# ShangHua-Gao/SOD100K

Hardware: NVIDIA H100
Metric: images/sec CSNet fwd 224x224 (higher is better)
Workload: dtype fp16

## Files before the change

### sod100k_b200/csrc/il_stream.cuh

```cuda
#pragma once
#include <cuda.h>

#include "il_block.cuh"

namespace csnet {

constexpr int kIlsMaxThreads = 384;
constexpr int kIlsMaxC = 64;
constexpr int kIlsHiStages = 2, kIlsLoStages = 3;

struct IlsArgs {
  void* yh;
  void* yl;
  const uint32_t* wh;
  const uint32_t* wl;
  DwParams dw1h, dw1l, dw2h, dw2l;
  float bias_h[kIlsMaxC], sm1_h[kIlsMaxC], bias_l[kIlsMaxC], sm1_l[kIlsMaxC];
  int32_t N, H, W;
  int32_t Chi, Cli, Cho, Clo;
  int32_t K8, K16, NH, NL;
  int32_t SH, SL, ST;
  int32_t GH, GL;
  int32_t ns, gsn, hl;
  int32_t GR, GLR;
  int32_t Ci, BW;
  int32_t off_xlo;
  int32_t cpi, total_chunks;
  int32_t dw_warps;
  int32_t hi_stage_bytes, lo_stage_bytes;
  int32_t off_xl, off_xh, off_t1l, off_wbh, off_wbl, off_bar, off_zero, off_epi, off_dwp, smem_bytes;
};

__device__ __forceinline__ void tma_load_5d(uint32_t dst, const CUtensorMap* tm, uint32_t bar, int c0, int c1, int c2, int c3, int c4) {
  asm volatile("cp.async.bulk.tensor.5d.shared::cluster.global.mbarrier::complete_tx::bytes [%0], [%1, {%3, %4, %5, %6, %7}], [%2];\n"
               ::"r"(dst), "l"(tm), "r"(bar), "r"(c0), "r"(c1), "r"(c2), "r"(c3), "r"(c4) : "memory");
}
__device__ __forceinline__ void tma_load_4d_a(uint32_t dst, const CUtensorMap* tm, uint32_t bar, int c0, int c1, int c2, int c3) {
  asm volatile("cp.async.bulk.tensor.4d.shared::cluster.global.mbarrier::complete_tx::bytes [%0], [%1, {%3, %4, %5, %6}], [%2];\n"
               ::"r"(dst), "l"(tm), "r"(bar), "r"(c0), "r"(c1), "r"(c2), "r"(c3) : "memory");
}
__device__ __forceinline__ void mbar_expect_tx_a(uint32_t bar, uint32_t bytes) {
  asm volatile("mbarrier.arrive.expect_tx.shared::cta.b64 _, [%0], %1;\n" ::"r"(bar), "r"(bytes) : "memory");
}
__device__ __forceinline__ void mbar_wait_a(uint32_t bar, uint32_t parity) {
  uint32_t ok = 0;
  const long long t0 = clock64();
  while (true) {
    asm volatile("{\n.reg .pred p;\nmbarrier.try_wait.parity.shared::cta.b64 p, [%1], %2;\nselp.u32 %0, 1, 0, p;\n}\n"
                 : "=r"(ok) : "r"(bar), "r"(parity) : "memory");
    if (ok) break;
    if (clock64() - t0 > 4000000000LL) __trap();
  }
}
__device__ __forceinline__ uint64_t gmma_desc(uint32_t saddr, uint32_t lbo_bytes, uint32_t sbo_bytes) {
// ... 51 lines not shown
                 : "l"(da), "l"(db), "r"(acc));
  }
  static __device__ __forceinline__ void mma0(float (&d)[32], uint64_t da, uint64_t db) {
    asm volatile("{\n.reg .pred p;\nsetp.ne.b32 p, %34, 0;\n"
                 "wgmma.mma_async.sync.aligned.m64n64k16.f32.f16.f16 {%0, %1, %2, %3, %4, %5, %6, %7, %8, %9, %10, %11, %12, %13, %14, %15, %16, %17, %18, %19, %20, %21, %22, %23, %24, %25, %26, %27, %28, %29, %30, %31}, %32, %33, p, 1, 1, 1, 0;\n}\n"
                 : "=f"(d[0]), "=f"(d[1]), "=f"(d[2]), "=f"(d[3]), "=f"(d[4]), "=f"(d[5]), "=f"(d[6]), "=f"(d[7]), "=f"(d[8]), "=f"(d[9]), "=f"(d[10]), "=f"(d[11]), "=f"(d[12]), "=f"(d[13]), "=f"(d[14]), "=f"(d[15]), "=f"(d[16]), "=f"(d[17]), "=f"(d[18]), "=f"(d[19]), "=f"(d[20]), "=f"(d[21]), "=f"(d[22]), "=f"(d[23]), "=f"(d[24]), "=f"(d[25]), "=f"(d[26]), "=f"(d[27]), "=f"(d[28]), "=f"(d[29]), "=f"(d[30]), "=f"(d[31])
                 : "l"(da), "l"(db), "r"(0u));
  }
};
template <> struct Wgmma<80> {
  static __device__ __forceinline__ void mma(float (&d)[40], uint64_t da, uint64_t db, uint32_t acc) {
    asm volatile("{\n.reg .pred p;\nsetp.ne.b32 p, %42, 0;\n"
                 "wgmma.mma_async.sync.aligned.m64n80k16.f32.f16.f16 {%0, %1, %2, %3, %4, %5, %6, %7, %8, %9, %10, %11, %12, %13, %14, %15, %16, %17, %18, %19, %20, %21, %22, %23, %24, %25, %26, %27, %28, %29, %30, %31, %32, %33, %34, %35, %36, %37, %38, %39}, %40, %41, p, 1, 1, 1, 0;\n}\n"
                 : "+f"(d[0]), "+f"(d[1]), "+f"(d[2]), "+f"(d[3]), "+f"(d[4]), "+f"(d[5]), "+f"(d[6]), "+f"(d[7]), "+f"(d[8]), "+f"(d[9]), "+f"(d[10]), "+f"(d[11]), "+f"(d[12]), "+f"(d[13]), "+f"(d[14]), "+f"(d[15]), "+f"(d[16]), "+f"(d[17]), "+f"(d[18]), "+f"(d[19]), "+f"(d[20]), "+f"(d[21]), "+f"(d[22]), "+f"(d[23]), "+f"(d[24]), "+f"(d[25]), "+f"(d[26]), "+f"(d[27]), "+f"(d[28]), "+f"(d[29]), "+f"(d[30]), "+f"(d[31]), "+f"(d[32]), "+f"(d[33]), "+f"(d[34]), "+f"(d[35]), "+f"(d[36]), "+f"(d[37]), "+f"(d[38]), "+f"(d[39])
                 : "l"(da), "l"(db), "r"(acc));
  }
  static __device__ __forceinline__ void mma0(float (&d)[40], uint64_t da, uint64_t db) {
    asm volatile("{\n.reg .pred p;\nsetp.ne.b32 p, %42, 0;\n"
                 "wgmma.mma_async.sync.aligned.m64n80k16.f32.f16.f16 {%0, %1, %2, %3, %4, %5, %6, %7, %8, %9, %10, %11, %12, %13, %14, %15, %16, %17, %18, %19, %20, %21, %22, %23, %24, %25, %26, %27, %28, %29, %30, %31, %32, %33, %34, %35, %36, %37, %38, %39}, %40, %41, p, 1, 1, 1, 0;\n}\n"
                 : "=f"(d[0]), "=f"(d[1]), "=f"(d[2]), "=f"(d[3]), "=f"(d[4]), "=f"(d[5]), "=f"(d[6]), "=f"(d[7]), "=f"(d[8]), "=f"(d[9]), "=f"(d[10]), "=f"(d[11]), "=f"(d[12]), "=f"(d[13]), "=f"(d[14]), "=f"(d[15]), "=f"(d[16]), "=f"(d[17]), "=f"(d[18]), "=f"(d[19]), "=f"(d[20]), "=f"(d[21]), "=f"(d[22]), "=f"(d[23]), "=f"(d[24]), "=f"(d[25]), "=f"(d[26]), "=f"(d[27]), "=f"(d[28]), "=f"(d[29]), "=f"(d[30]), "=f"(d[31]), "=f"(d[32]), "=f"(d[33]), "=f"(d[34]), "=f"(d[35]), "=f"(d[36]), "=f"(d[37]), "=f"(d[38]), "=f"(d[39])
                 : "l"(da), "l"(db), "r"(0u));
  }
};
__device__ __forceinline__ void wgmma_fence() { asm volatile("wgmma.fence.sync.aligned;\n" ::: "memory"); }
__device__ __forceinline__ void wgmma_commit_wait() {
  asm volatile("wgmma.commit_group.sync.aligned;\n" ::: "memory");
  asm volatile("wgmma.wait_group.sync.aligned 0;\n" ::: "memory");
}
__device__ __forceinline__ void warpgroup_bar(int wg) { asm volatile("bar.sync %0, 128;\n" ::"r"(1 + wg) : "memory"); }
template <int N>
__device__ __forceinline__ void wgmma_block(float (&d)[N / 2], uint64_t da, uint64_t db, int K16) {
  wgmma_fence();
  Wgmma<N>::mma0(d, da, db);
  for (int ks = 1; ks < (K16 >> 4); ++ks) Wgmma<N>::mma(d, da + (uint64_t)(16 * ks), db + (uint64_t)(16 * ks), 1u);
  wgmma_commit_wait();
}
__device__ __forceinline__ uint32_t lds32(uint32_t a) { uint32_t v; asm volatile("ld.shared.b32 %0, [%1];\n" : "=r"(v) : "r"(a)); return v; }
__device__ __forceinline__ uint2 lds64(uint32_t a) { uint2 v; asm volatile("ld.shared.v2.b32 {%0, %1}, [%2];\n" : "=r"(v.x), "=r"(v.y) : "r"(a)); return v; }
__device__ __forceinline__ uint4 lds128(uint32_t a) {
  uint4 v;
  asm volatile("ld.shared.v4.b32 {%0, %1, %2, %3}, [%4];\n" : "=r"(v.x), "=r"(v.y), "=r"(v.z), "=r"(v.w) : "r"(a));
  return v;
}
__device__ __forceinline__ uint16_t lds16(uint32_t a) { uint16_t v; asm volatile("ld.shared.u16 %0, [%1];\n" : "=h"(v) : "r"(a)); return v; }
__device__ __forceinline__ void sts128(uint32_t a, uint4 v) {
  asm volatile("st.shared.v4.b32 [%0], {%1, %2, %3, %4};\n" ::"r"(a), "r"(v.x), "r"(v.y), "r"(v.z), "r"(v.w) : "memory");
}
__device__ __forceinline__ void sts16(uint32_t a, uint16_t v) { asm volatile("st.shared.u16 [%0], %1;\n" ::"r"(a), "h"(v) : "memory"); }

__device__ __forceinline__ uint16_t h16(const uint32_t* row, int j) { return (j & 1) ? (uint16_t)(row[j >> 1] >> 16) : (uint16_t)row[j >> 1]; }

constexpr int kIlsDwpBytes = 96;
constexpr int kIlsTX = 20, kIlsT2 = 18, kIlsTO = 16;

template <int NO, bool kStart = false>
__device__ __forceinline__ void ils_dw_taps(float (&acc)[NO], const float* row, float4 w) {
#pragma unroll
  for (int i = 0; i < NO; ++i) {
    acc[i] = fmaf(row[i], w.x, kStart ? w.w : acc[i]);
// ... 46 lines not shown
  const float4 v1 = ils_dw_param(prm + 64u);
  ils_dw_taps<kIlsTO>(sob, q, v1);
  if (make_out) {
    uint32_t o[8];
#pragma unroll
    for (int k = 0; k < kIlsTO; k += 2) o[k >> 1] = Pack<T>::from_f2(prelu_m1(soa[k], v1.w), prelu_m1(soa[k + 1], v1.w));
    *reinterpret_cast<uint4*>(out) = make_uint4(o[0], o[1], o[2], o[3]);
    if (e.outB) *reinterpret_cast<uint4*>(out + 8) = make_uint4(o[4], o[5], o[6], o[7]);
  }
  ils_dw_taps<kIlsTO, true>(soa, q, ils_dw_param(prm + 48u));
  ils_dw_taps<kIlsT2, true>(s2a, x, ils_dw_param(prm));
}
template <typename T>
__device__ __forceinline__ void ils_dw_load(float (&x)[kIlsTX], uint32_t pA, uint32_t pB, uint32_t pL, uint32_t pR) {
  const uint4 a = lds128(pA), b = lds128(pB);
  const uint32_t u[10] = {lds32(pL), a.x, a.y, a.z, a.w, b.x, b.y, b.z, b.w, lds32(pR)};
#pragma unroll
  for (int i = 0; i < 10; ++i) {
    const float2 f = Pack<T>::to_f2(u[i]);
    x[2 * i] = f.x; x[2 * i + 1] = f.y;
  }
}

__device__ __forceinline__ void stsm_x4_trans(uint32_t addr, uint32_t a, uint32_t b, uint32_t c, uint32_t d) {
  asm volatile("stmatrix.sync.aligned.m8n8.x4.trans.shared.b16 [%0], {%1, %2, %3, %4};\n" ::"r"(addr), "r"(a), "r"(b), "r"(c), "r"(d) : "memory");
}

template <typename T, int N>
__device__ __forceinline__ void ils_block(uint64_t da, uint64_t db, int K16, int wg, uint32_t tile, uint32_t gstride, int g0, int ngroups,
                                          uint32_t eb, uint32_t es, uint32_t dummy, int lane) {
  float d[N / 2];
  wgmma_block<N>(d, da, db, K16);
  warpgroup_bar(wg);
  const int q = lane & 3, mrow = lane & 7, mat = lane >> 3;
#pragma unroll
  for (int cc = 0; cc < N / 16; ++cc) {
    const uint32_t co = (uint32_t)(cc * 16 + 2 * q) * 4u;
    const uint2 bA = lds64(eb + co), bB = lds64(eb + co + 32u), sA = lds64(es + co), sB = lds64(es + co + 32u);
    const float b0 = __uint_as_float(bA.x), b1 = __uint_as_float(bA.y), b2 = __uint_as_float(bB.x), b3 = __uint_as_float(bB.y);
    const float s0 = __uint_as_float(sA.x), s1 = __uint_as_float(sA.y), s2 = __uint_as_float(sB.x), s3 = __uint_as_float(sB.y);
    const float* r = d + 8 * cc;
    const uint32_t m0 = Pack<T>::from_f2(prelu_m1(r[0] + b0, s0), prelu_m1(r[1] + b1, s1));
    const uint32_t m1 = Pack<T>::from_f2(prelu_m1(r[2] + b0, s0), prelu_m1(r[3] + b1, s1));
    const uint32_t m2 = Pack<T>::from_f2(prelu_m1(r[4] + b2, s2), prelu_m1(r[5] + b3, s3));
    const uint32_t m3 = Pack<T>::from_f2(prelu_m1(r[6] + b2, s2), prelu_m1(r[7] + b3, s3));
    const int pg = g0 + (mat & 1);
    const uint32_t addr = pg < ngroups ? tile + (uint32_t)pg * gstride + (uint32_t)(cc * 16 + 8 * (mat >> 1) + mrow) * 16u
                                       : dummy + (uint32_t)(mat * 8 + mrow) * 16u;
    stsm_x4_trans(addr, m0, m1, m2, m3);
  }
}
template <typename T>
__device__ __forceinline__ void ils_block_n(int N, uint64_t da, uint64_t db, int K16, int wg, uint32_t tile, uint32_t gstride, int g0,
                                            int ngroups, uint32_t eb, uint32_t es, uint32_t dummy, int lane) {
  switch (N) {
    case 16: ils_block<T, 16>(da, db, K16, wg, tile, gstride, g0, ngroups, eb, es, dummy, lane); break;
    case 32: ils_block<T, 32>(da, db, K16, wg, tile, gstride, g0, ngroups, eb, es, dummy, lane); break;
    case 48: ils_block<T, 48>(da, db, K16, wg, tile, gstride, g0, ngroups, eb, es, dummy, lane); break;
    default: ils_block<T, 64>(da, db, K16, wg, tile, gstride, g0, ngroups, eb, es, dummy, lane); break;
  }
}

template <typename T, bool kStem = false>
__global__ void __launch_bounds__(kIlsMaxThreads, 1)
il_stream_kernel(const __grid_constant__ IlsArgs A, const __grid_constant__ CUtensorMap tmH, const __grid_constant__ CUtensorMap tmL) {
  extern __shared__ uint8_t smem_raw[];
  const int tid = threadIdx.x, lane = tid & 31, warp = tid >> 5, nthreads = blockDim.x, nwarps = nthreads >> 5;
  const uint32_t sbase = (smem_u32(smem_raw) + 127u) & ~127u;
  const uint32_t XL = sbase + A.off_xl, XH = sbase + A.off_xh, T1L = sbase + A.off_t1l, WBH = sbase + A.off_wbh,
                 WBL = sbase + A.off_wbl, BAR = sbase + A.off_bar, ZERO = sbase + A.off_zero;
  uint8_t* gbase = smem_raw + (sbase - smem_u32(smem_raw));
  const uint32_t bar_h = BAR, bar_l = BAR + 16;
  const uint32_t EPI = sbase + A.off_epi, DUMMY = EPI + 1024;

  const int H = A.H, W = A.W, Hl = H >> 1, Wl = W >> 1;
  const int Chi = A.Chi, Cli = A.Cli, Cho = A.Cho, Clo = A.Clo;
  const int GH = A.GH, GL = A.GL, SH = A.SH, SL = A.SL, ST = A.ST, NH = A.NH, NL = A.NL, K16 = A.K16;
  const int GR = A.GR, GLR = A.GLR, hl = A.hl, gsn = A.gsn;
  const int cpi = A.cpi;

  if (tid == 0) {
    for (int i = 0; i < 6; ++i) asm volatile("mbarrier.init.shared::cta.b64 [%0], 1;\n" ::"r"(BAR + 8 * i) : "memory");
// ... 45 lines not shown
  __syncthreads();

  const int n_hi_tasks = Cho * (gsn >> 1);
  const bool dw_hi = tid < n_hi_tasks;
  const int dwt = dw_hi ? tid : tid - n_hi_tasks;
  const int Gs = dw_hi ? gsn : gsn >> 1;
  const int Gd = (Gs + 1) >> 1, Cd = dw_hi ? Cho : Clo, Sd = dw_hi ? SH : ST;
  const bool dw_live = dwt < Cd * Gd;
  const int dc = dw_live ? dwt / Gd : 0, dg = dw_live ? 2 * (dwt - dc * Gd) : 0;
  const uint32_t prm = sbase + A.off_dwp + (uint32_t)((dw_hi ? dc : Cho + dc) * kIlsDwpBytes);
  const int dw_rows = dw_hi ? 4 : 2;
  const int dHd = dw_hi ? H : Hl, dWd = dw_hi ? W : Wl;
  const uint32_t dw_off = (uint32_t)((dg + hl) * Sd + dc) * 16u, dw_rowstep = (uint32_t)((dw_hi ? GR : GLR) * Sd) * 16u;
  const int Gimg = dw_hi ? GH : GL;

  const int nbh = (4 * GR + 7) >> 3, nbl = NL > 0 ? (2 * GLR + 7) >> 3 : 0;
  const uint64_t db_h = gmma_desc(WBH, 128u, (uint32_t)(K16 >> 3) * 128u), db_l = gmma_desc(WBL, 128u, (uint32_t)(K16 >> 3) * 128u);
  const uint32_t hi_tx = (uint32_t)(64 * SH * GR), lo_tx = kStem ? (uint32_t)(A.BW * 4 * A.Ci * 4) : (uint32_t)(32 * SL * GLR);
  const uint32_t XLO = sbase + A.off_xlo;

  int ra = (int)((long long)blockIdx.x * A.total_chunks / gridDim.x);
  const int rb = (int)((long long)(blockIdx.x + 1) * A.total_chunks / gridDim.x);
  uint32_t hq = 0, lq = 0;

  while (ra < rb) {
    const int item = ra / cpi, ca = ra - item * cpi;
    const int n = item / A.ns, gs0 = (item - n * A.ns) * gsn;
    const int cb = (ca + (rb - ra)) < cpi ? (ca + (rb - ra)) : cpi;
    ra += cb - ca;
    const int c0 = ca > 0 ? ca - 1 : 0, c1 = cb < cpi ? cb : cpi - 1;
    const int cl0 = c0 > 0 ? c0 - 1 : 0, cl1 = c1 + 1 < cpi ? c1 + 1 : cpi - 1;
    const int out_lo = dw_hi ? 4 * ca : 2 * ca, out_hi = dw_hi ? 4 * cb : 2 * cb;
    const uint32_t hq0 = hq, lq0 = lq;
    hq += (uint32_t)(c1 - c0 + 1);
    lq += (uint32_t)(cl1 - cl0 + 1);
    auto hi_stage = [&](int c) { return XH + ((hq0 + (uint32_t)(c - c0)) & 1u) * (uint32_t)A.hi_stage_bytes; };
    auto lo_stage = [&](int cl) { return XL + ((lq0 + (uint32_t)(cl - cl0)) % 3u) * (uint32_t)A.lo_stage_bytes; };
    auto issue_hi = [&](int c) {
      const uint32_t q = hq0 + (uint32_t)(c - c0), bar = bar_h + 8 * (q & 1u);
      mbar_expect_tx_a(bar, hi_tx);
      tma_load_5d(hi_stage(c), &tmH, bar, 0, 0, gs0 - hl, 4 * c, n);
    };
    auto issue_lo = [&](int cl) {
      const uint32_t q = lq0 + (uint32_t)(cl - cl0), bar = bar_l + 8 * (q % 3u);
      mbar_expect_tx_a(bar, lo_tx);
      if (kStem) tma_load_4d_a(lo_stage(cl), &tmL, bar, 8 * (gs0 - hl) - 4, 4 * cl, 0, n);
      else tma_load_5d(lo_stage(cl), &tmL, bar, 0, 0, (gs0 >> 1) - hl, 2 * cl, n);
    };
    if (tid == 0) {
      asm volatile("fence.proxy.async.shared::cta;\n" ::: "memory");
      if (!kStem) {
        issue_hi(c0);
        if (c0 + 1 <= c1) issue_hi(c0 + 1);
      }
      for (int cl = cl0; cl <= cl1 && cl <= c0 + 1; ++cl) issue_lo(cl);
    }
    int lo_waited = 0;
    IlsTail tl;
    if (dw_live) ils_dw_start(tl, prm);
    const int gimg = (dw_hi ? gs0 : gs0 >> 1) + dg;
    const bool hasB = gimg + 1 < Gimg, zeroL = gimg == 0, zeroR = gimg + 2 >= Gimg || dg + 2 >= Gs + hl;
    IlsTaskEdges edg;
    edg.m0 = zeroL ? 0.f : 1.f;
    edg.m9 = hasB ? 1.f : 0.f;
    edg.m17 = gimg + 2 >= Gimg ? 0.f : 1.f;
    edg.outB = dg + 1 < Gs;
    const uint32_t sd = (uint32_t)Sd * 16u;
    uint16_t* ybase = reinterpret_cast<uint16_t*>(dw_hi ? A.yh : A.yl) + ((size_t)n * Cd + dc) * dHd * dWd + 8 * gimg;

    for (int c = c0; c <= c1; ++c) {
      {
        const uint32_t q = hq0 + (uint32_t)(c - c0);
        if (!kStem) mbar_wait_a(bar_h + 8 * (q & 1u), (q >> 1) & 1u);
        const int need = (c + 1 < cpi ? c + 1 : cpi - 1) - cl0 + 1;
        while (lo_waited < need) {
          const uint32_t ql = lq0 + (uint32_t)lo_waited;
          mbar_wait_a(bar_l + 8 * (ql % 3u), (ql / 3u) & 1u);
          ++lo_waited;
        }
      }
      const uint32_t xh = hi_stage(c), xl = kStem ? XLO : lo_stage(c);
      if (kStem) {
        const int Ci = A.Ci, BW = A.BW;
        const int n_hi = 4 * GR * Ci * 3, n_lo = Clo > 0 ? 2 * GLR * Ci * 3 : 0;
        for (int task = tid; task < n_hi + n_lo; task += nthreads) {
          const bool hb = task < n_hi;
          const int t = hb ? task : task - n_hi, Gt = hb ? GR : GLR;
          const int ck = t % (Ci * 3), rg = t / (Ci * 3);
          const int ci = ck / 3, ky = ck - ci * 3, r = rg / Gt, g = rg - r * Gt;
          float f[10];
          if (hb) {
            const int yy = 4 * c + r + ky - 1;
            if (yy >= 0 && yy < H) {
              const uint32_t a = lo_stage(yy >> 2) + (uint32_t)(((ci * 4 + (yy & 3)) * BW + 8 * g + 3) * 4);
              const uint4 m0 = lds128(a + 4u), m1 = lds128(a + 20u);
              f[0] = __uint_as_float(lds32(a)); f[9] = __uint_as_float(lds32(a + 36u));
              f[1] = __uint_as_float(m0.x); f[2] = __uint_as_float(m0.y); f[3] = __uint_as_float(m0.z); f[4] = __uint_as_float(m0.w);
              f[5] = __uint_as_float(m1.x); f[6] = __uint_as_float(m1.y); f[7] = __uint_as_float(m1.z); f[8] = __uint_as_float(m1.w);
            } else {
#pragma unroll
              for (int j = 0; j < 10; ++j) f[j] = 0.f;
            }
          } else {
// ... 71 lines not shown
            const int ga = 2 * glr - hl;
            const bool okA = ga >= 0, okB = ga + 1 < GR;
            const uint32_t src = xh + (uint32_t)(ga * SH + ch) * 16u;
            const uint32_t dst = xl + (uint32_t)(glr * SL + Cli + ch) * 16u;
#pragma unroll
            for (int lr = 0; lr < 2; ++lr) {
              const uint32_t r0 = src + (uint32_t)(2 * lr * GR * SH) * 16u, r1 = r0 + (uint32_t)(GR * SH) * 16u;
              const uint4 a0 = lds128(okA ? r0 : ZERO), a1 = lds128(okB ? r0 + (uint32_t)SH * 16u : ZERO), c0_ = lds128(okA ? r1 : ZERO),
                          c1_ = lds128(okB ? r1 + (uint32_t)SH * 16u : ZERO);
              auto hmax = [](uint32_t u, uint32_t v) {
                return __byte_perm(Pack<T>::max2(u, __byte_perm(u, 0u, 0x1032)), Pack<T>::max2(v, __byte_perm(v, 0u, 0x1032)), 0x5410);
              };
              uint4 o;
              o.x = hmax(Pack<T>::max2(a0.x, c0_.x), Pack<T>::max2(a0.y, c0_.y));
              o.y = hmax(Pack<T>::max2(a0.z, c0_.z), Pack<T>::max2(a0.w, c0_.w));
              o.z = hmax(Pack<T>::max2(a1.x, c1_.x), Pack<T>::max2(a1.y, c1_.y));
              o.w = hmax(Pack<T>::max2(a1.z, c1_.z), Pack<T>::max2(a1.w, c1_.w));
              sts128(dst + (uint32_t)(lr * GLR * SL) * 16u, o);
            }
          }
        }
      }
      asm volatile("fence.proxy.async.shared::cta;\n" ::: "memory");
      __syncthreads();
      if (warp == nwarps - 1 && lane == 0) {
        asm volatile("fence.proxy.async.shared::cta;\n" ::: "memory");
        if (!kStem && c >= c0 + 1 && c + 1 <= c1) issue_hi(c + 1);
        if (c + 2 <= cl1) issue_lo(c + 2);
      }
      if (warp < (nwarps & ~3)) {
        const int wg = warp >> 2, qd = warp & 3, wgs = nwarps >> 2;
        for (int b = wg; b < nbh + nbl; b += wgs) {
          if (b < nbh)
            ils_block_n<T>(NH, gmma_desc(xh + (uint32_t)(b * 8 * SH) * 16u, 128u, (uint32_t)SH * 16u), db_h, K16, wg, xh, (uint32_t)SH * 16u,
                           b * 8 + qd * 2, 4 * GR, EPI, EPI + 256u, DUMMY, lane);
          else
            ils_block_n<T>(NL, gmma_desc(xl + (uint32_t)((b - nbh) * 8 * SL) * 16u, 128u, (uint32_t)SL * 16u), db_l, K16, wg, T1L,
                           (uint32_t)ST * 16u, (b - nbh) * 8 + qd * 2, 2 * GLR, EPI + 512u, EPI + 768u, DUMMY, lane);
        }
      }
      __syncthreads();
      if (dw_live) {
        const uint32_t t1b = (dw_hi ? xh : T1L) + dw_off;
        auto row = [&](float (&a2)[kIlsT2], float (&b2)[kIlsT2], float (&ao)[kIlsTO], float (&bo)[kIlsTO], int rr) {
          const int r = dw_rows * c + rr, tr = r - 1, orow = r - 2;
          const bool make_t2 = tr >= 0 && tr >= out_lo - 1 && tr <= out_hi;
          const bool make_out = orow >= out_lo && orow < out_hi;
          const uint32_t p = t1b + (uint32_t)rr * dw_rowstep;
          float x[kIlsTX];
          ils_dw_load<T>(x, p, hasB ? p + sd : ZERO, zeroL ? ZERO : p - sd + 12u, zeroR ? ZERO : p + 2u * sd);
          ils_dw_push<T>(a2, b2, ao, bo, x, prm, make_t2, edg, make_out, ybase + (size_t)orow * dWd);
        };
        for (int rr = 0; rr < dw_rows; rr += 2) {
          row(tl.s2a, tl.s2b, tl.soa, tl.sob, rr);
          row(tl.s2b, tl.s2a, tl.sob, tl.soa, rr + 1);
        }
      }
    }
    if (cb == cpi && dw_live) {
      float z[kIlsTX];
#pragma unroll
      for (int i = 0; i < kIlsTX; ++i) z[i] = 0.f;
      ils_dw_push<T>(tl.s2a, tl.s2b, tl.soa, tl.sob, z, prm, true, edg, dHd - 2 >= out_lo, ybase + (size_t)(dHd - 2) * dWd);
      ils_dw_push<T>(tl.s2b, tl.s2a, tl.sob, tl.soa, z, prm, false, edg, dHd - 1 >= out_lo, ybase + (size_t)(dHd - 1) * dWd);
    }
    __syncthreads();
  }
}

}
```

### sod100k_b200/csrc/plan.cu

```cuda
#include <cuda.h>
#include <cuda_runtime.h>

#include <cstdio>
#include <cstdlib>
#include <cstring>
#include <cstdint>
#include <new>
#include <string>
#include <vector>

#include "../../include/csnet_b200.h"
#include "generic_ops.cuh"
#include "il_block.cuh"
#include "il_stream.cuh"
#include "mix_stream.cuh"
#include "ms_direct.cuh"
#include "mix_tc.cuh"
#include "dw_fast.cuh"
#include "image_io.cuh"
#include "resize.cuh"
#include "resize_adj.cuh"

namespace {

// ... 465 lines not shown
  A.H = Yh.H; A.W = Yh.W;
  A.Chi = stem ? Xh.C * 9 : Xh.C; A.Cli = stem ? 0 : Xl.C; A.Cho = Yh.C; A.Clo = op.dst2 >= 0 ? P.tensors[op.dst2].C : 0;
  A.Ci = stem ? Xh.C : 0;
  if (stem && (Xh.dtype != CSNET_F32 || A.Chi > 32 || A.W % 4)) return false;
  if (A.W % 16 || A.H % 4 || A.Cho > csnet::kIlsMaxC || A.Clo > csnet::kIlsMaxC || A.Chi + A.Cli > 64) return false;
  A.K8 = stem ? 32 : round_up(A.Chi + A.Cli, 8);
  A.K16 = round_up(A.Chi + A.Cli, 16);
  A.NH = round_up(A.Cho, 16);
  A.NL = A.Clo > 0 ? round_up(A.Clo, 16) : 0;
  A.GH = A.W / 8; A.GL = A.W / 16;
  A.SH = (A.K16 > A.NH ? A.K16 : A.NH) + 1;
  A.SL = A.Clo > 0 ? A.K16 + 1 : (A.Cli | 1);
  A.ST = A.NL + 1;
  A.cpi = A.H / 4;
  auto r128 = [](int v) { return (v + 127) / 128 * 128; };
  bool found = false;
  csnet::IlsArgs best{};
  for (int ns = 1; ns <= 16; ++ns) {
    if (P.ils_force_ns > 0 && ns != P.ils_force_ns) continue;
    if (A.GH % ns || (A.GH / ns) % 2) continue;
    csnet::IlsArgs T = A;
    T.ns = ns; T.gsn = A.GH / ns; T.hl = ns > 1 ? 1 : 0;
    T.GR = T.gsn + 2 * T.hl; T.GLR = T.gsn / 2 + 2 * T.hl;
    T.dw_warps = (T.Cho * (T.gsn / 2) + T.Clo * ((T.gsn / 2 + 1) / 2) + 31) / 32;
    if (T.dw_warps < 4) T.dw_warps = 4;
    const int warps = T.dw_warps;
    if (warps * 32 > csnet::kIlsMaxThreads || T.SH > 256 || T.SL > 256 || T.GR > 256) continue;
    const int nbh = (4 * T.GR + 7) / 8, nbl = T.Clo > 0 ? (2 * T.GLR + 7) / 8 : 0;
    T.BW = 8 * T.GR + 8;
    if (stem && T.BW > 256) continue;
    T.lo_stage_bytes = stem ? r128(T.BW * 4 * T.Ci * 4) : r128(2 * T.GLR * T.SL * 16);
    T.hi_stage_bytes = r128(4 * T.GR * T.SH * 16);
    T.off_xl = 0;
    T.off_xh = csnet::kIlsLoStages * T.lo_stage_bytes;
    T.off_t1l = T.off_xh + csnet::kIlsHiStages * T.hi_stage_bytes;
    T.off_wbh = T.off_t1l + r128(2 * T.GLR * T.ST * 16);
    T.off_wbl = T.off_wbh + r128(T.NH * T.K16 * 2);
    T.off_bar = T.off_wbl + r128(T.NL * T.K16 * 2);
    T.off_zero = T.off_bar + 256;
    T.off_epi = T.off_zero + 128;
    T.off_dwp = T.off_epi + 1536;
    T.off_xlo = T.off_dwp + r128((T.Cho + T.Clo) * csnet::kIlsDwpBytes);
    int end = T.off_xlo + (stem ? r128(2 * T.GLR * T.SL * 16) : 0);
    const int over_h = T.off_xh + T.hi_stage_bytes + nbh * 8 * T.SH * 16,
              over_l = (stem ? T.off_xlo : T.off_xl + 2 * T.lo_stage_bytes) + nbl * 8 * T.SL * 16;
    end = over_h > end ? over_h : end;
    end = over_l > end ? over_l : end;
    T.smem_bytes = end + 128;
// ... 484 lines not shown
      break;
    }
    case Kern::Gn: {
      const csnet_tensor_desc& S = P->tensors[op.paths[0].src];
      csnet::GnArgs A{};
      A.src = P->tensor_ptr(op.paths[0].src, N, ext_ptrs);
      A.dst = P->tensor_ptr(op.dst, N, ext_ptrs);
      A.gamma = P->blob + op.ext_off[0];
      A.beta = P->blob + op.ext_off[1];
      A.slope = op.slope_off >= 0 ? P->blob + op.slope_off : nullptr;
      A.stats = P->gn_stats;
      A.src_dtype = S.dtype; A.dst_dtype = D.dtype; A.C = D.C; A.HW = D.H * D.W; A.groups = op.paths[0].up;
      gn_stats_kernel<<<dim3(A.groups, N), kThreads, 0, stream>>>(A);
      const int bx = (A.HW + kThreads * 4 - 1) / (kThreads * 4);
      gn_apply_kernel<<<dim3(bx < 1 ? 1 : bx, D.C, N), kThreads, 0, stream>>>(A);
      break;
    }
    case Kern::IlStream: {
      csnet::IlsArgs A = R.ils;
      A.yh = P->tensor_ptr(op.dst, N, ext_ptrs);
      A.yl = op.dst2 >= 0 ? P->tensor_ptr(op.dst2, N, ext_ptrs) : nullptr;
      A.N = N;
      A.total_chunks = N * A.ns * A.cpi;
      CUtensorMap tmH, tmL;
      const bool stem = A.Ci > 0;
      if (stem) {
        if (!encode_image_map(&tmL, P->tensor_ptr(op.paths[0].src, N, ext_ptrs), N, A.Ci, A.H, A.W, A.BW, 4, A.Ci))
          return fail(CSNET_E_CUDA, "cuTensorMapEncodeTiled failed (streaming ILBlock, image)");
        tmH = tmL;
      } else if (!encode_group_map(&tmH, P->tensor_ptr(op.paths[0].src, N, ext_ptrs), N, A.Chi, A.H, A.W, A.SH, A.GR, 4) ||
                 !encode_group_map(&tmL, P->tensor_ptr(op.paths[1].src, N, ext_ptrs), N, A.Cli, A.H / 2, A.W / 2, A.SL, A.GLR, 2))
        return fail(CSNET_E_CUDA, "cuTensorMapEncodeTiled failed (streaming ILBlock)");
      int grid = A.total_chunks / 4;
      grid = grid < 1 ? 1 : (grid > P->num_sms ? P->num_sms : grid);
      if (stem) csnet::il_stream_kernel<__half, true><<<grid, A.dw_warps * 32, A.smem_bytes, stream>>>(A, tmH, tmL);
      else csnet::il_stream_kernel<__half, false><<<grid, A.dw_warps * 32, A.smem_bytes, stream>>>(A, tmH, tmL);
      break;
    }
    case Kern::IlBlock: {
      csnet::IlArgs A = R.il;
      A.xh = P->tensor_ptr(op.paths[0].src, N, ext_ptrs);
      if (!A.first) A.xl = P->tensor_ptr(op.paths[1].src, N, ext_ptrs);
      A.yh = P->tensor_ptr(op.dst, N, ext_ptrs);
      if (op.dst2 >= 0) A.yl = P->tensor_ptr(op.dst2, N, ext_ptrs);
      const int tiles_y = (A.H + A.TH - 1) / A.TH;
      dim3 grid(A.tiles_x * tiles_y, 1, N);
// ... 126 lines not shown
}

void* csnet_plan_tensor_ptr(csnet_plan* P, int32_t tensor, int32_t N) {
  if (!P || tensor < 0 || tensor >= (int)P->tensors.size() || N <= 0 || N > P->max_batch) return nullptr;
  if (P->tensors[tensor].external >= 0) return nullptr;
  return P->tensor_ptr(tensor, N, nullptr);
}

int csnet_plan_read_tensor(csnet_plan* P, int32_t tensor, int32_t N, void* dst, void* stream) {
  void* src = csnet_plan_tensor_ptr(P, tensor, N);
  if (!src || !dst) return fail(CSNET_E_INVALID, "csnet_plan_read_tensor: bad tensor / batch / destination");
  const csnet_tensor_desc& d = P->tensors[tensor];
  DeviceGuard guard_(P->device);
  CU_CHECK(cudaMemcpyAsync(dst, src, (size_t)N * d.C * d.H * d.W * dtype_size(d.dtype), cudaMemcpyDeviceToDevice,
                           (cudaStream_t)stream));
  return CSNET_OK;
}

const char* csnet_plan_op_kernel(const csnet_plan* P, int32_t i) {
  if (!P || i < 0 || i >= (int32_t)P->ops.size()) return "";
  return kKernNames[(int)P->launch[i].kern];
}

int32_t csnet_plan_launches(const csnet_plan* P) {
  if (!P) return 0;
  int32_t n = 0;
  for (size_t i = 0; i < P->ops.size(); ++i)
    n += P->launch[i].kern == Kern::Gn ? 2 : (P->launch[i].kern == Kern::Msd ? P->ops[i].n_paths : 1);
  return n;
}

int64_t csnet_plan_arena_bytes(const csnet_plan* P) { return P ? P->arena_per_image * (int64_t)P->max_batch : 0; }

void csnet_plan_destroy(csnet_plan* P) {
  if (!P) return;
  drop_graphs(P);
  if (P->cap_stream) cudaStreamDestroy(P->cap_stream);
  DeviceGuard guard_(P->device);
  if (P->blob) cudaFree(P->blob);
  if (P->arena) cudaFree(P->arena);
  if (P->gn_stats) cudaFree(P->gn_stats);
  for (const OpLaunch& R : P->launch)
    for (uint16_t* q : R.w16)
      if (q) cudaFree(q);
  for (int b = 0; b < 2; ++b) {
    if (P->h_in[b]) cudaFree(P->h_in[b]);
// ... 326 lines not shown
```

Before: 18440.

## Switch streaming ILBlock GEMM to register-A wgmma via transposed ldmatrix

Replaces the shared-memory-descriptor wgmma for the A operand with register-sourced wgmma, loading A fragments per k-step with ldmatrix.trans. The block loop is split into separate hi and lo passes with their own warpgroup strides, and dw_warps is rounded up to a multiple of four so every warp joins a warpgroup. Compile-time-gated phase timing instrumentation is also added. Each k-step now does commit/wait serially, which may cost tensor-core overlap in exchange for avoiding the smem A layout constraint.

```diff
diff --git a/sod100k_b200/csrc/il_stream.cuh b/sod100k_b200/csrc/il_stream.cuh
--- a/sod100k_b200/csrc/il_stream.cuh
+++ b/sod100k_b200/csrc/il_stream.cuh
@@ -29,7 +29,24 @@
   int32_t dw_warps;
   int32_t hi_stage_bytes, lo_stage_bytes;
   int32_t off_xl, off_xh, off_t1l, off_wbh, off_wbl, off_bar, off_zero, off_epi, off_dwp, smem_bytes;
-};
+#ifdef CSNET_ILS_PHASES
+  int32_t phase_slot;
+#endif
+};
+
+#ifdef CSNET_ILS_PHASES
+enum IlsPhase { kPhWait, kPhResample, kPhBarA, kPhGemm, kPhBarB, kPhTail, kPhPiece, kIlsPhases };
+constexpr int kIlsPhaseSlots = 128;
+__device__ unsigned long long g_ils_phase[kIlsPhaseSlots][2][kIlsPhases + 1];
+#define ILS_MARK(k)                          \
+  do {                                       \
+    const uint32_t t_ = (uint32_t)clock();   \
+    ph_[k] += t_ - tp_;                      \
+    tp_ = t_;                                \
+  } while (0)
+#else
+#define ILS_MARK(k) do {} while (0)
+#endif
 
 __device__ __forceinline__ void tma_load_5d(uint32_t dst, const CUtensorMap* tm, uint32_t bar, int c0, int c1, int c2, int c3, int c4) {
   asm volatile("cp.async.bulk.tensor.5d.shared::cluster.global.mbarrier::complete_tx::bytes [%0], [%1, {%3, %4, %5, %6, %7}], [%2];\n"
@@ -127,19 +144,69 @@
                  : "l"(da), "l"(db), "r"(0u));
   }
 };
+template <int N> struct WgmmaRs;
+template <> struct WgmmaRs<16> {
+  static __device__ __forceinline__ void mma(float (&d)[8], const uint32_t (&a)[4], uint64_t db, uint32_t acc) {
+    asm volatile("{\n.reg .pred p;\nsetp.ne.b32 p, %13, 0;\n"
+                 "wgmma.mma_async.sync.aligned.m64n16k16.f32.f16.f16 {%0, %1, %2, %3, %4, %5, %6, %7}, {%8, %9, %10, %11}, %12, p, 1, 1, 0;\n}\n"
+                 : "+f"(d[0]), "+f"(d[1]), "+f"(d[2]), "+f"(d[3]), "+f"(d[4]), "+f"(d[5]), "+f"(d[6]), "+f"(d[7])
+                 : "r"(a[0]), "r"(a[1]), "r"(a[2]), "r"(a[3]), "l"(db), "r"(acc));
+  }
+  static __device__ __forceinline__ void mma0(float (&d)[8], const uint32_t (&a)[4], uint64_t db) {
+    asm volatile("{\n.reg .pred p;\nsetp.ne.b32 p, %13, 0;\n"
+                 "wgmma.mma_async.sync.aligned.m64n16k16.f32.f16.f16 {%0, %1, %2, %3, %4, %5, %6, %7}, {%8, %9, %10, %11}, %12, p, 1, 1, 0;\n}\n"
+                 : "=f"(d[0]), "=f"(d[1]), "=f"(d[2]), "=f"(d[3]), "=f"(d[4]), "=f"(d[5]), "=f"(d[6]), "=f"(d[7])
+                 : "r"(a[0]), "r"(a[1]), "r"(a[2]), "r"(a[3]), "l"(db), "r"(0u));
+  }
+};
+template <> struct WgmmaRs<32> {
+  static __device__ __forceinline__ void mma(float (&d)[16], const uint32_t (&a)[4], uint64_t db, uint32_t acc) {
+    asm volatile("{\n.reg .pred p;\nsetp.ne.b32 p, %21, 0;\n"
+                 "wgmma.mma_async.sync.aligned.m64n32k16.f32.f16.f16 {%0, %1, %2, %3, %4, %5, %6, %7, %8, %9, %10, %11, %12, %13, %14, %15}, {%16, %17, %18, %19}, %20, p, 1, 1, 0;\n}\n"
+                 : "+f"(d[0]), "+f"(d[1]), "+f"(d[2]), "+f"(d[3]), "+f"(d[4]), "+f"(d[5]), "+f"(d[6]), "+f"(d[7]), "+f"(d[8]), "+f"(d[9]), "+f"(d[10]), "+f"(d[11]), "+f"(d[12]), "+f"(d[13]), "+f"(d[14]), "+f"(d[15])
+                 : "r"(a[0]), "r"(a[1]), "r"(a[2]), "r"(a[3]), "l"(db), "r"(acc));
+  }
+  static __device__ __forceinline__ void mma0(float (&d)[16], const uint32_t (&a)[4], uint64_t db) {
+    asm volatile("{\n.reg .pred p;\nsetp.ne.b32 p, %21, 0;\n"
+                 "wgmma.mma_async.sync.aligned.m64n32k16.f32.f16.f16 {%0, %1, %2, %3, %4, %5, %6, %7, %8, %9, %10, %11, %12, %13, %14, %15}, {%16, %17, %18, %19}, %20, p, 1, 1, 0;\n}\n"
+                 : "=f"(d[0]), "=f"(d[1]), "=f"(d[2]), "=f"(d[3]), "=f"(d[4]), "=f"(d[5]), "=f"(d[6]), "=f"(d[7]), "=f"(d[8]), "=f"(d[9]), "=f"(d[10]), "=f"(d[11]), "=f"(d[12]), "=f"(d[13]), "=f"(d[14]), "=f"(d[15])
+                 : "r"(a[0]), "r"(a[1]), "r"(a[2]), "r"(a[3]), "l"(db), "r"(0u));
+  }
+};
+template <> struct WgmmaRs<48> {
+  static __device__ __forceinline__ void mma(float (&d)[24], const uint32_t (&a)[4], uint64_t db, uint32_t acc) {
+    asm volatile("{\n.reg .pred p;\nsetp.ne.b32 p, %29, 0;\n"
+                 "wgmma.mma_async.sync.aligned.m64n48k16.f32.f16.f16 {%0, %1, %2, %3, %4, %5, %6, %7, %8, %9, %10, %11, %12, %13, %14, %15, %16, %17, %18, %19, %20, %21, %22, %23}, {%24, %25, %26, %27}, %28, p, 1, 1, 0;\n}\n"
+                 : "+f"(d[0]), "+f"(d[1]), "+f"(d[2]), "+f"(d[3]), "+f"(d[4]), "+f"(d[5]), "+f"(d[6]), "+f"(d[7]), "+f"(d[8]), "+f"(d[9]), "+f"(d[10]), "+f"(d[11]), "+f"(d[12]), "+f"(d[13]), "+f"(d[14]), "+f"(d[15]), "+f"(d[16]), "+f"(d[17]), "+f"(d[18]), "+f"(d[19]), "+f"(d[20]), "+f"(d[21]), "+f"(d[22]), "+f"(d[23])
+                 : "r"(a[0]), "r"(a[1]), "r"(a[2]), "r"(a[3]), "l"(db), "r"(acc));
+  }
+  static __device__ __forceinline__ void mma0(float (&d)[24], const uint32_t (&a)[4], uint64_t db) {
+    asm volatile("{\n.reg .pred p;\nsetp.ne.b32 p, %29, 0;\n"
+                 "wgmma.mma_async.sync.aligned.m64n48k16.f32.f16.f16 {%0, %1, %2, %3, %4, %5, %6, %7, %8, %9, %10, %11, %12, %13, %14, %15, %16, %17, %18, %19, %20, %21, %22, %23}, {%24, %25, %26, %27}, %28, p, 1, 1, 0;\n}\n"
+                 : "=f"(d[0]), "=f"(d[1]), "=f"(d[2]), "=f"(d[3]), "=f"(d[4]), "=f"(d[5]), "=f"(d[6]), "=f"(d[7]), "=f"(d[8]), "=f"(d[9]), "=f"(d[10]), "=f"(d[11]), "=f"(d[12]), "=f"(d[13]), "=f"(d[14]), "=f"(d[15]), "=f"(d[16]), "=f"(d[17]), "=f"(d[18]), "=f"(d[19]), "=f"(d[20]), "=f"(d[21]), "=f"(d[22]), "=f"(d[23])
+                 : "r"(a[0]), "r"(a[1]), "r"(a[2]), "r"(a[3]), "l"(db), "r"(0u));
+  }
+};
+template <> struct WgmmaRs<64> {
+  static __device__ __forceinline__ void mma(float (&d)[32], const uint32_t (&a)[4], uint64_t db, uint32_t acc) {
+    asm volatile("{\n.reg .pred p;\nsetp.ne.b32 p, %37, 0;\n"
+                 "wgmma.mma_async.sync.aligned.m64n64k16.f32.f16.f16 {%0, %1, %2, %3, %4, %5, %6, %7, %8, %9, %10, %11, %12, %13, %14, %15, %16, %17, %18, %19, %20, %21, %22, %23, %24, %25, %26, %27, %28, %29, %30, %31}, {%32, %33, %34, %35}, %36, p, 1, 1, 0;\n}\n"
+                 : "+f"(d[0]), "+f"(d[1]), "+f"(d[2]), "+f"(d[3]), "+f"(d[4]), "+f"(d[5]), "+f"(d[6]), "+f"(d[7]), "+f"(d[8]), "+f"(d[9]), "+f"(d[10]), "+f"(d[11]), "+f"(d[12]), "+f"(d[13]), "+f"(d[14]), "+f"(d[15]), "+f"(d[16]), "+f"(d[17]), "+f"(d[18]), "+f"(d[19]), "+f"(d[20]), "+f"(d[21]), "+f"(d[22]), "+f"(d[23]), "+f"(d[24]), "+f"(d[25]), "+f"(d[26]), "+f"(d[27]), "+f"(d[28]), "+f"(d[29]), "+f"(d[30]), "+f"(d[31])
+                 : "r"(a[0]), "r"(a[1]), "r"(a[2]), "r"(a[3]), "l"(db), "r"(acc));
+  }
+  static __device__ __forceinline__ void mma0(float (&d)[32], const uint32_t (&a)[4], uint64_t db) {
+    asm volatile("{\n.reg .pred p;\nsetp.ne.b32 p, %37, 0;\n"
+                 "wgmma.mma_async.sync.aligned.m64n64k16.f32.f16.f16 {%0, %1, %2, %3, %4, %5, %6, %7, %8, %9, %10, %11, %12, %13, %14, %15, %16, %17, %18, %19, %20, %21, %22, %23, %24, %25, %26, %27, %28, %29, %30, %31}, {%32, %33, %34, %35}, %36, p, 1, 1, 0;\n}\n"
+                 : "=f"(d[0]), "=f"(d[1]), "=f"(d[2]), "=f"(d[3]), "=f"(d[4]), "=f"(d[5]), "=f"(d[6]), "=f"(d[7]), "=f"(d[8]), "=f"(d[9]), "=f"(d[10]), "=f"(d[11]), "=f"(d[12]), "=f"(d[13]), "=f"(d[14]), "=f"(d[15]), "=f"(d[16]), "=f"(d[17]), "=f"(d[18]), "=f"(d[19]), "=f"(d[20]), "=f"(d[21]), "=f"(d[22]), "=f"(d[23]), "=f"(d[24]), "=f"(d[25]), "=f"(d[26]), "=f"(d[27]), "=f"(d[28]), "=f"(d[29]), "=f"(d[30]), "=f"(d[31])
+                 : "r"(a[0]), "r"(a[1]), "r"(a[2]), "r"(a[3]), "l"(db), "r"(0u));
+  }
+};
 __device__ __forceinline__ void wgmma_fence() { asm volatile("wgmma.fence.sync.aligned;\n" ::: "memory"); }
 __device__ __forceinline__ void wgmma_commit_wait() {
   asm volatile("wgmma.commit_group.sync.aligned;\n" ::: "memory");
   asm volatile("wgmma.wait_group.sync.aligned 0;\n" ::: "memory");
 }
 __device__ __forceinline__ void warpgroup_bar(int wg) { asm volatile("bar.sync %0, 128;\n" ::"r"(1 + wg) : "memory"); }
-template <int N>
-__device__ __forceinline__ void wgmma_block(float (&d)[N / 2], uint64_t da, uint64_t db, int K16) {
-  wgmma_fence();
-  Wgmma<N>::mma0(d, da, db);
-  for (int ks = 1; ks < (K16 >> 4); ++ks) Wgmma<N>::mma(d, da + (uint64_t)(16 * ks), db + (uint64_t)(16 * ks), 1u);
-  wgmma_commit_wait();
-}
 __device__ __forceinline__ uint32_t lds32(uint32_t a) { uint32_t v; asm volatile("ld.shared.b32 %0, [%1];\n" : "=r"(v) : "r"(a)); return v; }
 __device__ __forceinline__ uint2 lds64(uint32_t a) { uint2 v; asm volatile("ld.shared.v2.b32 {%0, %1}, [%2];\n" : "=r"(v.x), "=r"(v.y) : "r"(a)); return v; }
 __device__ __forceinline__ uint4 lds128(uint32_t a) {
@@ -232,16 +299,17 @@
   }
 }
 
+__device__ __forceinline__ void ldsm_x4_trans(uint32_t addr, uint32_t (&a)[4]) {
+  asm volatile("ldmatrix.sync.aligned.m8n8.x4.trans.shared.b16 {%0, %1, %2, %3}, [%4];\n"
+               : "=r"(a[0]), "=r"(a[1]), "=r"(a[2]), "=r"(a[3]) : "r"(addr) : "memory");
+}
 __device__ __forceinline__ void stsm_x4_trans(uint32_t addr, uint32_t a, uint32_t b, uint32_t c, uint32_t d) {
   asm volatile("stmatrix.sync.aligned.m8n8.x4.trans.shared.b16 [%0], {%1, %2, %3, %4};\n" ::"r"(addr), "r"(a), "r"(b), "r"(c), "r"(d) : "memory");
 }
 
 template <typename T, int N>
-__device__ __forceinline__ void ils_block(uint64_t da, uint64_t db, int K16, int wg, uint32_t tile, uint32_t gstride, int g0, int ngroups,
-                                          uint32_t eb, uint32_t es, uint32_t dummy, int lane) {
-  float d[N / 2];
-  wgmma_block<N>(d, da, db, K16);
-  warpgroup_bar(wg);
+__device__ __forceinline__ void ils_epilogue(const float (&d)[N / 2], uint32_t tile, uint32_t gstride, int g0, int ngroups, uint32_t eb,
+                                             uint32_t es, uint32_t dummy, int lane) {
   const int q = lane & 3, mrow = lane & 7, mat = lane >> 3;
 #pragma unroll
   for (int cc = 0; cc < N / 16; ++cc) {
@@ -260,14 +328,37 @@
     stsm_x4_trans(addr, m0, m1, m2, m3);
   }
 }
+template <typename T, int N>
+__device__ __forceinline__ void ils_gemm(int b0, int b1, int bs, uint32_t at, uint32_t astride, uint64_t db, int K16, int wg, uint32_t tile,
+                                         uint32_t gstride, int qd, int ngroups, uint32_t eb, uint32_t es, uint32_t dummy, int lane) {
+  for (int b = b0; b < b1; b += bs) {
+    const int m = lane >> 3;
+    const uint32_t pa = at + (uint32_t)(8 * b + 2 * qd + (m & 1)) * astride + (uint32_t)(8 * (m >> 1) + (lane & 7)) * 16u;
+    float d[N / 2];
+    uint32_t a[4];
+    ldsm_x4_trans(pa, a);
+    wgmma_fence();
+    WgmmaRs<N>::mma0(d, a, db);
+    wgmma_commit_wait();
+    for (int ks = 1; ks < (K16 >> 4); ++ks) {
+      ldsm_x4_trans(pa + (uint32_t)(256 * ks), a);
+      wgmma_fence();
+      WgmmaRs<N>::mma(d, a, db + (uint64_t)(16 * ks), 1u);
+      wgmma_commit_wait();
+    }
+    warpgroup_bar(wg);
+    ils_epilogue<T, N>(d, tile, gstride, 8 * b + 2 * qd, ngroups, eb, es, dummy, lane);
+  }
+}
 template <typename T>
-__device__ __forceinline__ void ils_block_n(int N, uint64_t da, uint64_t db, int K16, int wg, uint32_t tile, uint32_t gstride, int g0,
-                                            int ngroups, uint32_t eb, uint32_t es, uint32_t dummy, int lane) {
+__device__ __forceinline__ void ils_gemm_n(int N, int b0, int b1, int bs, uint32_t at, uint32_t astride, uint64_t db, int K16, int wg,
+                                           uint32_t tile, uint32_t gstride, int qd, int ngroups, uint32_t eb, uint32_t es, uint32_t dummy,
+                                           int lane) {
   switch (N) {
-    case 16: ils_block<T, 16>(da, db, K16, wg, tile, gstride, g0, ngroups, eb, es, dummy, lane); break;
-    case 32: ils_block<T, 32>(da, db, K16, wg, tile, gstride, g0, ngroups, eb, es, dummy, lane); break;
-    case 48: ils_block<T, 48>(da, db, K16, wg, tile, gstride, g0, ngroups, eb, es, dummy, lane); break;
-    default: ils_block<T, 64>(da, db, K16, wg, tile, gstride, g0, ngroups, eb, es, dummy, lane); break;
+    case 16: ils_gemm<T, 16>(b0, b1, bs, at, astride, db, K16, wg, tile, gstride, qd, ngroups, eb, es, dummy, lane); break;
+    case 32: ils_gemm<T, 32>(b0, b1, bs, at, astride, db, K16, wg, tile, gstride, qd, ngroups, eb, es, dummy, lane); break;
+    case 48: ils_gemm<T, 48>(b0, b1, bs, at, astride, db, K16, wg, tile, gstride, qd, ngroups, eb, es, dummy, lane); break;
+    default: ils_gemm<T, 64>(b0, b1, bs, at, astride, db, K16, wg, tile, gstride, qd, ngroups, eb, es, dummy, lane); break;
   }
 }
 
@@ -359,6 +450,9 @@
   int ra = (int)((long long)blockIdx.x * A.total_chunks / gridDim.x);
   const int rb = (int)((long long)(blockIdx.x + 1) * A.total_chunks / gridDim.x);
   uint32_t hq = 0, lq = 0;
+#ifdef CSNET_ILS_PHASES
+  uint32_t ph_[kIlsPhases] = {}, tp_ = (uint32_t)clock(), walked_ = 0;
+#endif
 
   while (ra < rb) {
     const int item = ra / cpi, ca = ra - item * cpi;
@@ -405,7 +499,11 @@
     const uint32_t sd = (uint32_t)Sd * 16u;
     uint16_t* ybase = reinterpret_cast<uint16_t*>(dw_hi ? A.yh : A.yl) + ((size_t)n * Cd + dc) * dHd * dWd + 8 * gimg;
 
+#ifdef CSNET_ILS_PHASES
+    walked_ += (uint32_t)(c1 - c0 + 1);
+#endif
     for (int c = c0; c <= c1; ++c) {
+      if (c == c0) ILS_MARK(kPhPiece);
       {
         const uint32_t q = hq0 + (uint32_t)(c - c0);
         if (!kStem) mbar_wait_a(bar_h + 8 * (q & 1u), (q >> 1) & 1u);
@@ -416,6 +514,7 @@
           ++lo_waited;
         }
       }
+      ILS_MARK(kPhWait);
       const uint32_t xh = hi_stage(c), xl = kStem ? XLO : lo_stage(c);
       if (kStem) {
         const int Ci = A.Ci, BW = A.BW;
@@ -533,7 +632,9 @@
         }
       }
       asm volatile("fence.proxy.async.shared::cta;\n" ::: "memory");
+      ILS_MARK(kPhResample);
       __syncthreads();
+      ILS_MARK(kPhBarA);
       if (warp == nwarps - 1 && lane == 0) {
         asm volatile("fence.proxy.async.shared::cta;\n" ::: "memory");
         if (!kStem && c >= c0 + 1 && c + 1 <= c1) issue_hi(c + 1);
@@ -541,16 +642,15 @@
       }
       if (warp < (nwarps & ~3)) {
         const int wg = warp >> 2, qd = warp & 3, wgs = nwarps >> 2;
-        for (int b = wg; b < nbh + nbl; b += wgs) {
-          if (b < nbh)
-            ils_block_n<T>(NH, gmma_desc(xh + (uint32_t)(b * 8 * SH) * 16u, 128u, (uint32_t)SH * 16u), db_h, K16, wg, xh, (uint32_t)SH * 16u,
-                           b * 8 + qd * 2, 4 * GR, EPI, EPI + 256u, DUMMY, lane);
-          else
-            ils_block_n<T>(NL, gmma_desc(xl + (uint32_t)((b - nbh) * 8 * SL) * 16u, 128u, (uint32_t)SL * 16u), db_l, K16, wg, T1L,
-                           (uint32_t)ST * 16u, (b - nbh) * 8 + qd * 2, 2 * GLR, EPI + 512u, EPI + 768u, DUMMY, lane);
-        }
-      }
+#pragma unroll 1
+        for (int lo = 0; lo < (nbl > 0 ? 2 : 1); ++lo)
+          ils_gemm_n<T>(lo ? NL : NH, lo ? ((wg - nbh) % wgs + wgs) % wgs : wg, lo ? nbl : nbh, wgs, lo ? xl : xh, (uint32_t)(lo ? SL : SH) * 16u,
+                        lo ? db_l : db_h, K16, wg, lo ? T1L : xh, (uint32_t)(lo ? ST : SH) * 16u, qd, lo ? 2 * GLR : 4 * GR,
+                        EPI + (lo ? 512u : 0u), EPI + (lo ? 768u : 256u), DUMMY, lane);
+      }
+      ILS_MARK(kPhGemm);
       __syncthreads();
+      ILS_MARK(kPhBarB);
       if (dw_live) {
         const uint32_t t1b = (dw_hi ? xh : T1L) + dw_off;
         auto row = [&](float (&a2)[kIlsT2], float (&b2)[kIlsT2], float (&ao)[kIlsTO], float (&bo)[kIlsTO], int rr) {
@@ -567,6 +667,7 @@
           row(tl.s2b, tl.s2a, tl.sob, tl.soa, rr + 1);
         }
       }
+      ILS_MARK(kPhTail);
     }
     if (cb == cpi && dw_live) {
       float z[kIlsTX];
@@ -577,6 +678,14 @@
     }
     __syncthreads();
   }
-}
-
-}
+#ifdef CSNET_ILS_PHASES
+  ILS_MARK(kPhPiece);
+  if (lane == 0) {
+    unsigned long long* row = g_ils_phase[A.phase_slot][warp < (nwarps & ~3) ? 0 : 1];
+    for (int k = 0; k < kIlsPhases; ++k) atomicAdd(row + k, (unsigned long long)ph_[k]);
+    atomicAdd(row + kIlsPhases, (unsigned long long)walked_);
+  }
+#endif
+}
+
+}
diff --git a/sod100k_b200/csrc/plan.cu b/sod100k_b200/csrc/plan.cu
--- a/sod100k_b200/csrc/plan.cu
+++ b/sod100k_b200/csrc/plan.cu
@@ -511,8 +511,7 @@
     csnet::IlsArgs T = A;
     T.ns = ns; T.gsn = A.GH / ns; T.hl = ns > 1 ? 1 : 0;
     T.GR = T.gsn + 2 * T.hl; T.GLR = T.gsn / 2 + 2 * T.hl;
-    T.dw_warps = (T.Cho * (T.gsn / 2) + T.Clo * ((T.gsn / 2 + 1) / 2) + 31) / 32;
-    if (T.dw_warps < 4) T.dw_warps = 4;
+    T.dw_warps = ((T.Cho * (T.gsn / 2) + T.Clo * ((T.gsn / 2 + 1) / 2) + 31) / 32 + 3) / 4 * 4;
     const int warps = T.dw_warps;
     if (warps * 32 > csnet::kIlsMaxThreads || T.SH > 256 || T.SL > 256 || T.GR > 256) continue;
     const int nbh = (4 * T.GR + 7) / 8, nbl = T.Clo > 0 ? (2 * T.GLR + 7) / 8 : 0;
@@ -1043,6 +1042,9 @@
       A.yl = op.dst2 >= 0 ? P->tensor_ptr(op.dst2, N, ext_ptrs) : nullptr;
       A.N = N;
       A.total_chunks = N * A.ns * A.cpi;
+#ifdef CSNET_ILS_PHASES
+      A.phase_slot = (int32_t)i < csnet::kIlsPhaseSlots ? (int32_t)i : csnet::kIlsPhaseSlots - 1;
+#endif
       CUtensorMap tmH, tmL;
       const bool stem = A.Ci > 0;
       if (stem) {
@@ -1215,6 +1217,18 @@
   return kKernNames[(int)P->launch[i].kern];
 }
 
+#ifdef CSNET_ILS_PHASES
+int csnet_ils_phases(unsigned long long* out, int32_t n) {
+  constexpr int kN = csnet::kIlsPhaseSlots * 2 * (csnet::kIlsPhases + 1);
+  if (!out || n != kN) return fail(CSNET_E_INVALID, "csnet_ils_phases: size");
+  static const unsigned long long zero[kN] = {};
+  CU_CHECK(cudaDeviceSynchronize());
+  CU_CHECK(cudaMemcpyFromSymbol(out, csnet::g_ils_phase, sizeof zero));
+  CU_CHECK(cudaMemcpyToSymbol(csnet::g_ils_phase, zero, sizeof zero));
+  return CSNET_OK;
+}
+#endif
+
 int32_t csnet_plan_launches(const csnet_plan* P) {
   if (!P) return 0;
   int32_t n = 0;
```

Result: no change. 18550, median of 6 (+0.6%).
